# jabberjabberjabber/video-3d-pipeline

Hardware: AMD Instinct MI355X
Metric: 1080p_sbs_to_4k_depth_frames_per_s (higher is better)
Workload: dtype int16 (SGM) + f64 (guided filter sums; f32 depth in/out)

## Files before the change

### video-3d-pipeline_amd/csrc/v3d_common.h

```cpp
#pragma once
#include <hip/hip_runtime.h>
#include <stdint.h>
#include <stdio.h>
#include <stdarg.h>
#include "../../include/v3d_hip.h"

#define V3D_D 64
#define V3D_MAX_COST 32767
#define V3D_INVALID16 (-16)

void v3d_set_error(const char* fmt, ...);

struct v3d_lib_options {
    int gf_band1, gf_band2;
    int gf_tiled;
    int gf_fused;
    int gf_band;
    int gf_cols;
    int gf_int1;
    int corr_gather;
    int corr_fused;
};
extern v3d_lib_options g_v3d_opt;

#define V3D_HIP_CHECK(expr)                                                              \
    do {                                                                                 \
        hipError_t _e = (expr);                                                          \
        if (_e != hipSuccess) {                                                          \
            v3d_set_error("%s failed: %s (%s:%d)", #expr, hipGetErrorString(_e), __FILE__, __LINE__); \
            (void)hipGetLastError();    \
            return V3D_ERR_HIP;                                                          \
        }                                                                                \
    } while (0)

#define V3D_LAUNCH_CHECK()                                                               \
    do {                                                                                 \
        hipError_t _e = hipGetLastError();                                               \
        if (_e != hipSuccess) {                                                          \
            v3d_set_error("kernel launch failed: %s (%s:%d)", hipGetErrorString(_e), __FILE__, __LINE__); \
            return V3D_ERR_HIP;                                                          \
        }                                                                                \
    } while (0)

static inline int v3d_cdiv(int a, int b) { return (a + b - 1) / b; }

#ifdef __HIPCC__
typedef short v3d_s16x2 __attribute__((ext_vector_type(2)));
typedef unsigned short v3d_u16x2 __attribute__((ext_vector_type(2)));

__device__ __forceinline__ v3d_s16x2 as_s(uint32_t a) { return __builtin_bit_cast(v3d_s16x2, a); }
__device__ __forceinline__ v3d_u16x2 as_us(uint32_t a) { return __builtin_bit_cast(v3d_u16x2, a); }
__device__ __forceinline__ uint32_t as_u(v3d_s16x2 a) { return __builtin_bit_cast(uint32_t, a); }
__device__ __forceinline__ uint32_t as_u(v3d_u16x2 a) { return __builtin_bit_cast(uint32_t, a); }

__device__ __forceinline__ uint32_t pk_min(uint32_t a, uint32_t b) { return as_u(__builtin_elementwise_min(as_s(a), as_s(b))); }
__device__ __forceinline__ uint32_t pk_max(uint32_t a, uint32_t b) { return as_u(__builtin_elementwise_max(as_s(a), as_s(b))); }
__device__ __forceinline__ uint32_t pk_add(uint32_t a, uint32_t b) { return as_u((v3d_s16x2)(as_s(a) + as_s(b))); }
__device__ __forceinline__ uint32_t pk_sub(uint32_t a, uint32_t b) { return as_u((v3d_s16x2)(as_s(a) - as_s(b))); }
__device__ __forceinline__ uint32_t pk_add_sat(uint32_t a, uint32_t b) { return as_u(__builtin_elementwise_add_sat(as_s(a), as_s(b))); }
__device__ __forceinline__ uint32_t pk_subu_sat(uint32_t a, uint32_t b) { return as_u(__builtin_elementwise_sub_sat(as_us(a), as_us(b))); }
__device__ __forceinline__ uint32_t pk_minu(uint32_t a, uint32_t b) { return as_u(__builtin_elementwise_min(as_us(a), as_us(b))); }
__device__ __forceinline__ uint32_t pk_shr_u(uint32_t a, int n) { return as_u((v3d_u16x2)(as_us(a) >> (unsigned short)n)); }
__device__ __forceinline__ uint32_t pk_bcast(int v) { return ((uint32_t)v & 0xFFFFu) * 0x00010001u; }

__device__ __forceinline__ uint32_t alignbit(uint32_t hi, uint32_t lo, uint32_t sh) { return __builtin_amdgcn_alignbit(hi, lo, sh); }

#define V3D_DPP_QUAD(a, b, c, d) ((a) | ((b) << 2) | ((c) << 4) | ((d) << 6))
#define V3D_DPP_ROW_SHL(n) (0x100 + (n))
#define V3D_DPP_ROW_SHR(n) (0x110 + (n))
#define V3D_DPP_ROW_MIRROR 0x140
#define V3D_DPP_ROW_HALF_MIRROR 0x141

template <int CTRL>
__device__ __forceinline__ uint32_t dpp_mov(uint32_t old, uint32_t src)
{
    return (uint32_t)__builtin_amdgcn_update_dpp((int)old, (int)src, CTRL, 0xF, 0xF, false);
}
template <int CTRL>
__device__ __forceinline__ uint32_t dpp_xchg(uint32_t src)
{
    return (uint32_t)__builtin_amdgcn_update_dpp(0, (int)src, CTRL, 0xF, 0xF, true);
}
#ifndef V3D_NT
#define V3D_NT 1
#endif
typedef uint32_t v3d_u32x4 __attribute__((ext_vector_type(4)));
typedef uint32_t v3d_u32x2 __attribute__((ext_vector_type(2)));
__device__ __forceinline__ uint4 ld_stream(const uint4* p)
{
#if V3D_NT
    const v3d_u32x4 v = __builtin_nontemporal_load(reinterpret_cast<const v3d_u32x4*>(p));
    return make_uint4(v.x, v.y, v.z, v.w);
#else
    return *p;
#endif
}
__device__ __forceinline__ uint2 ld_stream(const uint2* p)
{
#if V3D_NT
    const v3d_u32x2 v = __builtin_nontemporal_load(reinterpret_cast<const v3d_u32x2*>(p));
    return make_uint2(v.x, v.y);
#else
    return *p;
#endif
}
__device__ __forceinline__ void st_stream(uint4* p, uint4 v)
{
#if V3D_NT
    v3d_u32x4 t = { v.x, v.y, v.z, v.w };
    __builtin_nontemporal_store(t, reinterpret_cast<v3d_u32x4*>(p));
#else
// ... 44 lines not shown
```

### video-3d-pipeline_amd/csrc/v3d_sgbm.hip

```cpp
#include "v3d_common.h"
#include <vector>
#include <string.h>
#include <type_traits>

#ifndef V3D_CK_NT
#define V3D_CK_NT 1
#endif
#ifndef V3D_C12
#define V3D_C12 1
#endif
#ifndef V3D_X_SPLIT
#define V3D_X_SPLIT 0
#endif
#define VOL_PX V3D_D
__host__ __device__ static inline size_t vol_row(int y, int W1) { return (size_t)y * W1 * V3D_D; }
__host__ __device__ static inline size_t vol_frame(int H, int W1) { return (size_t)H * W1 * V3D_D; }
#define C_PXB (V3D_C12 ? 96 : 128)
__host__ __device__ static inline size_t c_row(int y, int W1) { return (size_t)y * W1 * C_PXB; }
__host__ __device__ static inline size_t c_frame(int H, int W1) { return (size_t)H * W1 * C_PXB; }

#ifndef PF_BAND
#define PF_BAND 64
#endif
__global__ __launch_bounds__(256) void k_prefilter(const uint8_t* __restrict__ img1, const uint8_t* __restrict__ img2,
// ... 220 lines not shown
#pragma unroll
                for (int j = 0; j < NP; j++) V[i][j] = pr[j];
            }
#pragma unroll
            for (int j = 0; j < NP; j++) {
                const uint32_t c = bt_pair(U[0], U[1], U[2], V[0][j], V[1][j], V[2][j]);
                pix[j] = pl == 0 ? c : pix[j] + pk_shr_u(c, 2);
            }
            if (pl == 0) { if (NP == 4) asm volatile("" : "+v"(pix[0]), "+v"(pix[1]), "+v"(pix[NP - 2]), "+v"(pix[NP - 1]) :: "memory");
                           else asm volatile("" : "+v"(pix[0]), "+v"(pix[NP - 1]) :: "memory"); }
        }
        sPix[buf][col][dq] = Packer<NP>::go(pix);

        if (k + 1 < nrows && ld_any) stage(buf ^ 1, nr[buf ^ 1]);
        nr[buf ^ 1] = fetch(k + 3);
        __syncthreads();

        {
            uint32_t h[NP], w[NP];
            vec_unpack<NP>(sPix[buf][hc - 2][dq], h);
#pragma unroll
            for (int t = -1; t <= 2; t++) {
                vec_unpack<NP>(sPix[buf][hc + t][dq], w);
#pragma unroll
                for (int j = 0; j < NP; j++) h[j] += w[j];
            }
#pragma unroll
            for (int j = 0; j < NP; j++) { vs[j] += h[j] - ring[slot][j]; ring[slot][j] = h[j]; }
            const uint32_t st_row = k >= 4 ? (uint32_t)c_row(ys + k - 4, W1) : V3D_BUF_OOB;
            const uint32_t st_off = __builtin_elementwise_add_sat(st_col, st_row);
#if V3D_C12
            {
                uint32_t t[NP];
#pragma unroll
                for (int j = 0; j < NP; j++)
                    asm("v_bfi_b32 %0, %1, %2, %3" : "=v"(t[j]) : "s"(0xFFFu), "v"(vs[j]), "v"(vs[j] >> 4));
                const v3d_u32x3_a4 pk = { __builtin_amdgcn_perm(t[1], t[0], 0x04020100u), __builtin_amdgcn_perm(t[2], t[1], 0x05040201u),
                                          __builtin_amdgcn_perm(t[NP - 1], t[2], 0x06050402u) };
                __builtin_amdgcn_raw_buffer_store_b96(pk, rs_c, st_off, 0, V3D_NT ? 2 : 0);
            }
#else
            buf_store_stream(rs_c, st_off, Packer<NP>::go(vs));
#endif
        }
      }
    }
}

struct ChainArgs {
    const unsigned char* C; int16_t* S;
    int W1, H, W, nframes;
    int P1, P2;
    int uniq;
    uint32_t* wta;
    int xcd;
    int persist;
    int* ticket;
};

template <int LPP>
__device__ __forceinline__ uint32_t pk_hmin_lanes(uint32_t mn)
{
    uint32_t m1;
    asm("v_pk_min_u16 %0, %1, %1 op_sel:[0,1] op_sel_hi:[1,0]" : "=v"(m1) : "v"(mn));
    m1 = min(m1, dpp_xchg<V3D_DPP_QUAD(1, 0, 3, 2)>(m1));
    m1 = min(m1, dpp_xchg<V3D_DPP_QUAD(2, 3, 0, 1)>(m1));
    if (LPP >= 8) m1 = min(m1, dpp_xchg<V3D_DPP_ROW_HALF_MIRROR>(m1));
    if (LPP >= 16) m1 = min(m1, dpp_xchg<V3D_DPP_ROW_MIRROR>(m1));
    return m1;
}

template <int NP, int LPP>
__device__ __forceinline__ uint32_t chain_step(const uint32_t (&p)[NP], uint32_t delta, const uint32_t (&c)[NP],
                                               uint32_t (&L)[NP], uint32_t P1pk, uint32_t P2pk, bool first_lane, bool last_lane)
{
    const uint32_t MAXPK = 0x7FFF7FFFu;
    const uint32_t fill_prev = first_lane ? MAXPK : 0u, fill_next = last_lane ? MAXPK : 0u;
    const uint32_t prev = dpp_xchg<V3D_DPP_ROW_SHR(1)>(p[NP - 1]) | fill_prev;
    const uint32_t next = dpp_xchg<V3D_DPP_ROW_SHL(1)>(p[0]) | fill_next;
    uint32_t m[NP + 1];
    m[0] = alignbit(p[0], prev, 16);
#pragma unroll
    for (int i = 1; i < NP; i++) m[i] = alignbit(p[i], p[i - 1], 16);
    m[NP] = alignbit(next, p[NP - 1], 16);
    uint32_t mn = MAXPK;
#pragma unroll
    for (int i = 0; i < NP; i++) {
        uint32_t n = pk_add(pk_min(m[i], m[i + 1]), P1pk);
        L[i] = pk_sub(c[i], pk_subu_sat(delta, pk_min(p[i], n)));
        mn = pk_min(mn, L[i]);
    }
    return pk_add(pk_hmin_lanes<LPP>(mn), P2pk);
}

template <int NP, int LPP>
__device__ __forceinline__ uint32_t chain_delta(const uint32_t (&p)[NP], uint32_t P2pk)
{
    uint32_t mn = p[0];
#pragma unroll
    for (int i = 1; i < NP; i++) mn = pk_min(mn, p[i]);
    return pk_add(pk_hmin_lanes<LPP>(mn), P2pk);
}

#define WTA_ROWB 144

__device__ __forceinline__ uint32_t wta_word(int minS, int d16, int best) { return ((uint32_t)minS << 17) | ((uint32_t)(d16 + 16) << 6) | (uint32_t)best; }
__device__ __forceinline__ int wta_d16(uint32_t w) { return (int)((w >> 6) & 0x7FFu) - 16; }

__device__ __forceinline__ void wta_pixel(const unsigned char* srow, bool valid, int x, int y, int frame,
                                          const ChainArgs& a)
{
    uint32_t v[32];
#pragma unroll
    for (int q = 0; q < 8; q++) {
        const uint4 t = *reinterpret_cast<const uint4*>(srow + q * 16);
        v[4 * q] = t.x; v[4 * q + 1] = t.y; v[4 * q + 2] = t.z; v[4 * q + 3] = t.w;
    }
    uint32_t mpk = v[0];
#pragma unroll
    for (int i = 1; i < 32; i++) mpk = pk_minu(mpk, v[i]);
    const int minS = (int)min(mpk & 0xFFFFu, mpk >> 16);
    const uint32_t minpk = pk_bcast(minS), k64 = 0x00400040u;
    uint32_t kacc = 0xFFFFFFFFu;
#pragma unroll
    for (int i = 0; i < 32; i++) {
        uint32_t key;
        const uint32_t t = pk_subu_sat(v[i], minpk), dc = (uint32_t)(2 * i) | ((uint32_t)(2 * i + 1) << 16);
        asm("v_pk_mad_u16 %0, %1, %2, %3 clamp" : "=v"(key) : "v"(t), "v"(k64), "s"(dc));
        kacc = pk_minu(kacc, key);
    }
    const int best = (int)(min(kacc & 0xFFFFu, kacc >> 16) & 63u);
    const int uq = 100 - a.uniq, thr = minS * 100;
    int T1 = uq > 0 ? (thr + uq - 1) / uq : (thr > 0 ? 32768 : 0);
    T1 = min(T1, 32768);
    const uint32_t T1pk = pk_bcast(T1), one = 0x00010001u;
    uint32_t cntpk = 0;
#pragma unroll
    for (int i = 0; i < 32; i++) cntpk += pk_minu(pk_subu_sat(T1pk, v[i]), one);
    const int cnt = (int)(cntpk & 0xFFFFu) + (int)(cntpk >> 16);
    const unsigned short* s16 = reinterpret_cast<const unsigned short*>(srow);
    const int sm = best > 0 ? (int)s16[best - 1] : 0, sp = best < V3D_D - 1 ? (int)s16[best + 1] : 0;
    int cw = (minS < T1) ? 1 : 0;
    if (best > 0 && sm < T1) cw++;
    if (best < V3D_D - 1 && sp < T1) cw++;
    const bool ok = valid && (minS < V3D_MAX_COST) && (cnt <= cw);
    if (!valid) return;
    uint32_t word = 0u;
    if (ok) {
        int d16 = best * 16;
        if (best > 0 && best < V3D_D - 1) {
            const int den = max(sm + sp - 2 * minS, 1);
            d16 += ((sm - sp) * 16 + den) / (den * 2);
        }
        word = wta_word(minS, d16, best);
    }
    a.wta[((size_t)frame * a.H + y) * a.W + x + V3D_D] = word;
}

template <bool HORIZ, int XS, bool YREV, int MODE, int DPL>
__global__ __launch_bounds__(256) void k_chain(ChainArgs a)
{
    constexpr int NP = DPL / 2, LPP = 64 / DPL, PPW = DPL;
    constexpr int PF = 4;
    constexpr int BS = 64 / PPW;
    typedef typename VecT<DPL>::type Vec;
    static_assert(MODE != 2 || HORIZ, "the WTA tail rides on a horizontal direction");

    __shared__ __attribute__((aligned(16))) unsigned char sS[MODE == 2 ? 4 * 64 * WTA_ROWB : 16];

    const int lane = threadIdx.x & 63, wib = threadIdx.x >> 6;
    const int W1 = a.W1, H = a.H;
    const int NC = HORIZ ? H : (XS == 0 ? W1 : W1 + H - 1);
    const int groups = (NC + PPW - 1) / PPW;
    const int gw = blockIdx.x * 4 + wib;
    const int frame = gw / groups, grp = gw - frame * groups;
    if (frame >= a.nframes) return;

    const int sub = lane / LPP, dl = lane % LPP;
    const int c0 = grp * PPW, c1 = min(c0 + PPW, NC) - 1;
    const int c = c0 + sub;
    const bool cvalid = c <= c1;
    const int cc = min(c, c1);

    int tlo = 0, thi;
    if (HORIZ) thi = W1;
    else if (XS == 0) thi = H;
    else if (XS > 0) { tlo = max(0, H - 1 - c1); thi = min(H, W1 + H - 1 - c0); }
    else { tlo = max(0, c0 - (W1 - 1)); thi = min(H, c1 + 1); }

    const unsigned char* Cf = a.C + (size_t)frame * c_frame(H, W1) + c_lane_off<DPL>(dl);
    int16_t* Sf = a.S + (size_t)frame * vol_frame(H, W1) + dl * DPL;
    const int x0 = HORIZ ? 0 : (XS == 0 ? cc : (XS > 0 ? cc - (H - 1) : cc));

    auto pos = [&](int t, int& x, int& y) {
        if (HORIZ) { x = XS > 0 ? t : W1 - 1 - t; y = cc; }
        else { y = YREV ? H - 1 - t : t; x = x0 + XS * t; }
    };
    auto pix_off = [&](int t) -> int {
        int x, y; pos(t, x, y);
        x = min(max(x, 0), W1 - 1);
        return y * W1 + x;
    };

    const uint32_t P1pk = pk_bcast(a.P1), P2pk = pk_bcast(a.P2);
    const bool first_lane = dl == 0, last_lane = dl == LPP - 1;

    uint32_t p[NP];
#pragma unroll
    for (int i = 0; i < NP; i++) p[i] = 0;
// ... 28 lines not shown
                bool active = cvalid;
                if (!HORIZ && XS != 0) {
                    int x, y; pos(t, x, y);
                    active = cvalid && ((unsigned)x < (unsigned)W1);
#pragma unroll
                    for (int i = 0; i < NP; i++) L[i] = active ? L[i] : 0u;
                    nd = active ? nd : P2pk;
                }
#pragma unroll
                for (int i = 0; i < NP; i++) p[i] = L[i];
                delta = nd;
                if (MODE == 0) {
                    if (active) *reinterpret_cast<Vec*>(Sf + o) = Packer<NP>::go(L);
                } else {
#pragma unroll
                    for (int i = 0; i < NP; i++) sv[i] = pk_add_sat(sv[i], L[i]);
                    if (MODE == 1) {
                        if (active) *reinterpret_cast<Vec*>(Sf + o) = Packer<NP>::go(sv);
                    } else {
                        *reinterpret_cast<Vec*>(myS + (sub * BS + jj) * WTA_ROWB + dl * DPL * 2) = Packer<NP>::go(sv);
                    }
                }
            }
        }
        if (MODE == 2) {
            const int wsub = lane / BS, wj = lane % BS;
            const int t = tb + wj;
            const int y = c0 + wsub;
            const int x = XS > 0 ? t : W1 - 1 - t;
            const bool valid = (y <= c1) && (t < thi);
            wta_pixel(myS + lane * WTA_ROWB, valid, x, y, frame, a);
        }
    }
}

template <int DPL> struct HfC {
    typedef typename CRaw<DPL>::type Raw;
    static __device__ __forceinline__ const unsigned char* base(const unsigned char* C, int frame, int H, int W1, int row, int dl)
    {
        return C + (size_t)frame * c_frame(H, W1) + c_row(row, W1) + c_lane_off<DPL>(dl);
    }
    static __device__ __forceinline__ Raw load(const unsigned char* b, int x) { return c_load<DPL, !V3D_C12>(b + (size_t)x * C_PXB); }
};

template <int DPL>
__device__ __forceinline__ void hf_phase1(const unsigned char* Crow, uint32_t* ck, int nblk, int dl, uint32_t P1pk, uint32_t P2pk)
{
    constexpr int NP = DPL / 2, LPP = 64 / DPL, K = 64 / DPL;
    const bool first_lane = dl == 0, last_lane = dl == LPP - 1;
    uint32_t p[NP];
#pragma unroll
    for (int i = 0; i < NP; i++) p[i] = 0;
    uint32_t delta = P2pk;
    const int xend = (nblk - 1) * K;
    for (int xb = 0; xb < xend; xb += K) {
        typename HfC<DPL>::Raw cb[K];
#pragma unroll
        for (int jj = 0; jj < K; jj++) cb[jj] = HfC<DPL>::load(Crow, xb + jj);
#pragma unroll
        for (int jj = 0; jj < K; jj++) {
            uint32_t cv[NP], L[NP];
            vec_unpack<NP>(c_unpack(cb[jj], dl, P2pk), cv);
            delta = chain_step<NP, LPP>(p, delta, cv, L, P1pk, P2pk, first_lane, last_lane);
#pragma unroll
            for (int i = 0; i < NP; i++) p[i] = L[i];
        }
        uint32_t* c = ck + (size_t)(xb / K + 1) * NP * 64;
#pragma unroll
        for (int i = 0; i < NP; i++) { if (V3D_CK_NT) __builtin_nontemporal_store(p[i], c + i * 64); else c[i * 64] = p[i]; }
    }
}

template <int DPL, int PH>
__global__ __launch_bounds__(256, 4) void k_hfused(ChainArgs a, uint32_t* __restrict__ ckpt)
{
    constexpr int NP = DPL / 2, LPP = 64 / DPL, PPW = DPL, K = 64 / PPW;
    typedef typename VecT<DPL>::type Vec;
    __shared__ __attribute__((aligned(16))) unsigned char sS[4 * 64 * WTA_ROWB];

    const int lane = threadIdx.x & 63, wib = threadIdx.x >> 6;
    const int W1 = a.W1, H = a.H;
    const int groups = (H + PPW - 1) / PPW, total = groups * a.nframes;
    const int sub = lane / LPP, dl = lane % LPP;
    const int nblk = (W1 + K - 1) / K;
    const uint32_t P1pk = pk_bcast(a.P1), P2pk = pk_bcast(a.P2);
    const bool first_lane = dl == 0, last_lane = dl == LPP - 1;
    unsigned char* myS = sS + wib * 64 * WTA_ROWB;
    auto draw = [&]() -> int {
        int g = 0;
        if (lane == 0) g = atomicAdd(a.ticket, 1);
        return __builtin_amdgcn_readfirstlane(g);
    };
    int work = a.persist ? draw() : (a.xcd ? (int)xcd_linear(blockIdx.x, gridDim.x) : (int)blockIdx.x) * 4 + wib;
    for (;;) {
    if (work >= total) break;
    {
    const int frame = work / groups, grp = work - frame * groups;
    const int c0 = grp * PPW, c1 = min(c0 + PPW, H) - 1;
    const int cc = min(c0 + sub, c1);
    const unsigned char* Crow = HfC<DPL>::base(a.C, frame, H, W1, cc, dl);
    const int16_t* Srow = a.S + (size_t)frame * vol_frame(H, W1) + vol_row(cc, W1) + dl * DPL;
    uint32_t* ck = ckpt + ((size_t)frame * groups + grp) * nblk * NP * 64 + lane;
    if (PH & 1) hf_phase1<DPL>(Crow, ck, nblk, dl, P1pk, P2pk);

    uint32_t q[NP];
#pragma unroll
    for (int i = 0; i < NP; i++) q[i] = 0;
    uint32_t qdelta = P2pk;
    for (int blk = nblk - 1; blk >= 0; blk--) {
        const int x0 = blk * K;
        typename HfC<DPL>::Raw craw[K]; Vec cvv[K], svv[K];
#pragma unroll
        for (int j = 0; j < K; j++) {
            const int xj = min(x0 + j, W1 - 1);
            craw[j] = HfC<DPL>::load(Crow, xj);
            svv[j] = ld_stream(reinterpret_cast<const Vec*>(Srow + (size_t)xj * VOL_PX));
        }
        uint32_t p[NP], delta = P2pk;
#pragma unroll
        for (int i = 0; i < NP; i++) p[i] = 0;
        if (blk > 0) {
            const uint32_t* c = ck + (size_t)blk * NP * 64;
#pragma unroll
            for (int i = 0; i < NP; i++) p[i] = V3D_CK_NT ? __builtin_nontemporal_load(c + i * 64) : c[i * 64];
            delta = chain_delta<NP, LPP>(p, P2pk);
        }
        uint32_t L0[K][NP];
#pragma unroll
        for (int j = 0; j < K; j++) {
            uint32_t cv[NP];
            cvv[j] = c_unpack(craw[j], dl, P2pk);
            vec_unpack<NP>(cvv[j], cv);
            delta = chain_step<NP, LPP>(p, delta, cv, L0[j], P1pk, P2pk, first_lane, last_lane);
#pragma unroll
            for (int i = 0; i < NP; i++) p[i] = L0[j][i];
        }
#pragma unroll
        for (int jj = 0; jj < K; jj++) {
            const int j = K - 1 - jj;
            if (x0 + j < W1) {
                uint32_t cv[NP], sv[NP], L[NP];
                vec_unpack<NP>(cvv[j], cv);
                vec_unpack<NP>(svv[j], sv);
                qdelta = chain_step<NP, LPP>(q, qdelta, cv, L, P1pk, P2pk, first_lane, last_lane);
#pragma unroll
                for (int i = 0; i < NP; i++) { q[i] = L[i]; sv[i] = pk_add_sat(pk_add_sat(sv[i], L0[j][i]), L[i]); }
                *reinterpret_cast<Vec*>(myS + (sub * K + jj) * WTA_ROWB + dl * DPL * 2) = Packer<NP>::go(sv);
            }
        }
        {
            const int wsub = lane / K, wj = lane % K;
            const int x = x0 + K - 1 - wj, y = c0 + wsub;
            wta_pixel(myS + lane * WTA_ROWB, (y <= c1) && (x < W1), x, y, frame, a);
        }
    }
    }
    if (!a.persist) break;
    work = draw();
    }
}

template <int DPL>
__global__ __launch_bounds__(256, 8) void k_hscan(ChainArgs a, uint32_t* __restrict__ ckpt)
{
    constexpr int NP = DPL / 2, LPP = 64 / DPL, PPW = DPL, K = 64 / PPW;
    const int lane = threadIdx.x & 63, wib = threadIdx.x >> 6;
    const int W1 = a.W1, H = a.H;
    const int groups = (H + PPW - 1) / PPW;
    const int gw = (int)blockIdx.x * 4 + wib;
    const int frame = gw / groups, grp = gw - frame * groups;
    if (frame >= a.nframes) return;
    const int sub = lane / LPP, dl = lane % LPP;
    const int c0 = grp * PPW, c1 = min(c0 + PPW, H) - 1;
    const int cc = min(c0 + sub, c1);
    const int nblk = (W1 + K - 1) / K;
    uint32_t* ck = ckpt + ((size_t)frame * groups + grp) * nblk * NP * 64 + lane;
    hf_phase1<DPL>(HfC<DPL>::base(a.C, frame, H, W1, cc, dl), ck, nblk, dl, pk_bcast(a.P1), pk_bcast(a.P2));
}

#define VDD_RING 4
#define VDD_GRAN 34
#define VDD_SPIN_PER_ROW 64
#define VDD_SPIN_SLACK 4096

struct VddArgs {
    const unsigned char* C; int16_t* S;
    int W1, H, nframes, nstrips;
    int P1, P2;
    uint32_t seq;
    int spin_limit;
    unsigned long long* gran;
    int* err;
    int xcd;
};

template <int N>
__device__ __forceinline__ bool vdd_poll_n(const unsigned long long* g, const unsigned long long* gd, bool want_d,
                                           uint32_t tag, uint32_t (&v)[N], uint32_t& vd, int& budget)
{
    for (;;) {
        unsigned long long x[N], xd = (unsigned long long)tag << 32;
#pragma unroll
        for (int i = 0; i < N; i++) x[i] = __hip_atomic_load(g + i, __ATOMIC_RELAXED, __HIP_MEMORY_SCOPE_AGENT);
        if (want_d) xd = __hip_atomic_load(gd, __ATOMIC_RELAXED, __HIP_MEMORY_SCOPE_AGENT);
        bool ok = (uint32_t)(xd >> 32) == tag;
#pragma unroll
        for (int i = 0; i < N; i++) ok = ok && ((uint32_t)(x[i] >> 32) == tag);
        if (ok) {
// ... 533 lines not shown
}

__global__ __launch_bounds__(256) void k_ccl_apply(int16_t* __restrict__ img, int W, int H, int newVal, int maxSize,
                                                   const int* __restrict__ lab, const int* __restrict__ runs, const int* __restrict__ csz)
{
    const int y = blockIdx.x * 4 + (threadIdx.x >> 6), lane = threadIdx.x & 63;
    if (y >= H) return;
    const size_t fo = (size_t)blockIdx.z * W * H;
    const int* L = lab + fo;
    const int* rl = runs + fo + (size_t)y * W;
    const int row_end = (y + 1) * W;
    for (int k0 = 0; k0 < W; k0 += 64) {
        const int k = k0 + lane;
        const int s = k < W ? rl[k] : -1;
        const unsigned long long endm = __builtin_amdgcn_ballot_w64(s < 0);
        const int first_end = endm ? __builtin_ctzll(endm) : 64;
        if (lane < first_end) {
            const int r = ccl_find(L, s);
            if (csz[fo + r] <= maxSize) {
                img[fo + s] = (int16_t)newVal;
                for (int i = s + 1; i < row_end && L[i] == s; i++) img[fo + i] = (int16_t)newVal;
            }
        }
        if (first_end < 64) break;
    }
}

static int launch_speckles(int16_t* img, int W, int H, int frames, int newVal, int maxSize, int maxDiff, int32_t* ws, hipStream_t st)
{
    const int px = W * H;
    int* lab = ws; int* runs = ws + (size_t)px * frames; int* csz = ws + (size_t)px * frames * 2;
    hipLaunchKernelGGL(k_ccl_runs, dim3(v3d_cdiv(H, 4), 1, frames), dim3(256), 0, st, img, W, H, newVal, maxDiff, lab, runs, csz);
    hipLaunchKernelGGL(k_ccl_vmerge<0>, dim3(v3d_cdiv(W, 512), H - H / VM_BAND, frames), dim3(64), 0, st, img, W, H, newVal, maxDiff, lab);
    if (H / VM_BAND > 0) hipLaunchKernelGGL(k_ccl_vmerge<1>, dim3(v3d_cdiv(W, 512), H / VM_BAND, frames), dim3(64), 0, st, img, W, H, newVal, maxDiff, lab);
    hipLaunchKernelGGL(k_ccl_count, dim3(v3d_cdiv(H, 4), 1, frames), dim3(256), 0, st, W, H, maxSize, lab, runs, csz);
    hipLaunchKernelGGL(k_ccl_apply, dim3(v3d_cdiv(H, 4), 1, frames), dim3(256), 0, st, img, W, H, newVal, maxSize, lab, runs, csz);
    V3D_LAUNCH_CHECK();
    return V3D_OK;
}

__global__ __launch_bounds__(256) void k_c_export(const unsigned char* __restrict__ C, size_t npx, int P2, int16_t* __restrict__ out)
{
    const size_t i = (size_t)blockIdx.x * 256 + threadIdx.x, px = i >> 3;
    const int dl = (int)(i & 7);
    if (px >= npx) return;
    const uint4 v = c_unpack(*reinterpret_cast<const typename CRaw<8>::type*>(C + px * C_PXB + c_lane_off<8>(dl)), dl, pk_bcast(P2));
    *reinterpret_cast<uint4*>(out + px * V3D_D + 8 * dl) = v;
}

struct v3d_sgbm {
    v3d_sgbm_params prm;
    int device, maxW, maxH, maxB;
    int P1, P2, ftzero, uniq, d12;
    int dpl;
    uint4* rec;
    unsigned char* C;
    int16_t* S;
    uint32_t* wta;
    uint32_t* ckpt;
    unsigned long long* gran;
    size_t gran_bytes;
    int* vdd_err;
    uint32_t vdd_seq;
    int vdd_mode;
    int vdd_dpl;
    int cost_band;
    int vdd_xcd, cost_xcd, hf_xcd;
    int lrm_tiles;
    int hf_persist;
    int* hf_ticket;
    int vdd_mf4, vdd_mf8;
    int vdd_occ4, vdd_occ8, ncu;
    int reserve_cus;
    int vdd_launch_frames;
    int vdd_spin_limit;
    int* err_host;
    hipEvent_t vdd_done_ev;
    bool vdd_ev_recorded;
    bool hfused;
    int hsplit;
    int32_t* labels;
    size_t bytes;
    bool prof_on;
    int prof_calls;
    std::vector<hipEvent_t> prof_ev;
};

enum { ST_PREFILTER = 0, ST_COST, ST_V2, ST_D1, ST_D3, ST_H0, ST_V2R, ST_D1R, ST_D3R, ST_H4_WTA, ST_LRCHECK, ST_MEDIAN, ST_SPECKLE, V3D_NSTAGE };
static const char* const g_stage_names[V3D_NSTAGE] = { "prefilter", "cost", "chain_v2", "chain_d1", "chain_d3", "chain_h0",
    "chain_v2r", "chain_d1r", "chain_d3r", "chain_h4_wta", "lrcheck", "median", "speckles" };
#define V3D_PROF_MAX_CALLS 512

static inline void prof_mark(v3d_sgbm* h, int slot, hipStream_t stm)
{
    if (!h->prof_on || h->prof_calls >= V3D_PROF_MAX_CALLS) return;
    (void)hipEventRecord(h->prof_ev[(size_t)h->prof_calls * (V3D_NSTAGE + 1) + slot], stm);
}

extern "C" void v3d_sgbm_default_params(v3d_sgbm_params* p)
{
    p->minDisparity = 0; p->numDisparities = 64; p->blockSize = 5; p->P1 = 8 * 3 * 25; p->P2 = 32 * 3 * 25;
    p->disp12MaxDiff = 1; p->preFilterCap = 0; p->uniquenessRatio = 10; p->speckleWindowSize = 100;
    p->speckleRange = 32; p->mode = V3D_MODE_SGBM;
}

template <typename T> static int ws_alloc(T** p, size_t n, size_t* total)
// ... 31 lines not shown
    else if (is("vdd_xcd")) { if (value != 0 && value != 1) return bad(); h->vdd_xcd = value; }
    else if (is("hf_xcd")) { if (value != 0 && value != 1) return bad(); h->hf_xcd = value; }
    else if (is("hf_persist")) { if (value != 0 && value != 1) return bad(); h->hf_persist = value; }
    else if (is("lrm_tiles")) { if (value != 0 && value != 1) return bad(); h->lrm_tiles = value; }
    else if (is("reserve_cus")) { if (value < 0 || value > h->ncu) return bad(); h->reserve_cus = value; vdd_size_launches(h); }
    else if (is("vdd_spin_limit")) { if (value < -1) return bad(); h->vdd_spin_limit = value; }
    else if (is("vdd_launch_frames")) { if (value < 0) return bad(); h->vdd_launch_frames = value; }
    else { v3d_set_error("unknown option %s", key); return V3D_ERR_ARG; }
    return V3D_OK;
}
extern "C" int v3d_sgbm_get_option(const v3d_sgbm* h, const char* key, int* value)
{
    if (!h || !key || !value) { v3d_set_error("null argument"); return V3D_ERR_ARG; }
    auto is = [&](const char* k) { return strcmp(key, k) == 0; };
    if (is("lockstep")) *value = vdd_usable(h) ? 1 : 0;
    else if (is("hfused")) *value = h->hfused ? 1 : 0;
    else if (is("chain_dpl")) *value = h->dpl;
    else if (is("hsplit")) *value = h->hsplit;
    else if (is("vdd_dpl")) *value = h->vdd_dpl;
    else if (is("cost_band")) *value = h->cost_band;
    else if (is("cost_xcd")) *value = h->cost_xcd;
    else if (is("vdd_xcd")) *value = h->vdd_xcd;
    else if (is("hf_xcd")) *value = h->hf_xcd;
    else if (is("hf_persist")) *value = h->hf_persist;
    else if (is("lrm_tiles")) *value = h->lrm_tiles;
    else if (is("reserve_cus")) *value = h->reserve_cus;
    else if (is("vdd_spin_limit")) *value = h->vdd_spin_limit;
    else if (is("vdd_launch_frames")) *value = h->vdd_launch_frames;
    else if (is("vdd_frames_per_launch_dpl4")) *value = h->vdd_mf4;
    else if (is("vdd_frames_per_launch_dpl8")) *value = h->vdd_mf8;
    else { v3d_set_error("unknown option %s", key); return V3D_ERR_ARG; }
    return V3D_OK;
}

extern "C" int v3d_sgbm_create(const v3d_sgbm_params* prm, int device, int maxW, int maxH, int maxB, v3d_sgbm** out)
{
    if (!prm || !out) { v3d_set_error("null argument"); return V3D_ERR_ARG; }
    if (prm->minDisparity != 0 || prm->numDisparities != V3D_D || prm->blockSize != 5) {
        v3d_set_error("this build supports minDisparity=0, numDisparities=64, blockSize=5 (got %d, %d, %d)",
                      prm->minDisparity, prm->numDisparities, prm->blockSize);
        return V3D_ERR_UNSUPPORTED;
    }
    if (prm->mode != V3D_MODE_SGBM && prm->mode != V3D_MODE_HH) { v3d_set_error("unsupported mode %d", prm->mode); return V3D_ERR_UNSUPPORTED; }
    if (maxW <= V3D_D + 4 || maxH < 1 || maxB < 1) { v3d_set_error("bad geometry %dx%d batch %d", maxW, maxH, maxB); return V3D_ERR_ARG; }
    if ((size_t)maxW * maxH * V3D_D >= ((size_t)1 << 30)) { v3d_set_error("frame too large for 31-bit volume byte offsets"); return V3D_ERR_UNSUPPORTED; }
    V3D_HIP_CHECK(hipSetDevice(device));
    v3d_sgbm* h = new v3d_sgbm();
    h->prof_on = false; h->prof_calls = 0;
    h->prm = *prm; h->device = device; h->maxW = maxW; h->maxH = maxH; h->maxB = maxB;
    h->P1 = prm->P1 > 0 ? prm->P1 : 2;
    h->P2 = prm->P2 > 0 ? prm->P2 : 5; if (h->P2 < h->P1 + 1) h->P2 = h->P1 + 1;
    h->ftzero = (prm->preFilterCap > 15 ? prm->preFilterCap : 15) | 1;
    h->uniq = prm->uniquenessRatio >= 0 ? prm->uniquenessRatio : 10;
    h->d12 = prm->disp12MaxDiff > 0 ? prm->disp12MaxDiff : 1;
    if (2 * h->P2 + 25 * (2 * h->ftzero + 63) >= 32767 || h->ftzero > 31) {
        const int p2 = h->P2; delete h;
        v3d_set_error("P2=%d / preFilterCap exceed the int16 range of the packed SGM recurrence (need 2*P2 + 25*(2*ftzero+63) < 32767)", p2);
        return V3D_ERR_UNSUPPORTED;
    }
    h->dpl = 4;
    const size_t px = (size_t)maxW * maxH * maxB, vol = vol_frame(maxH, maxW - V3D_D) * maxB;
    h->bytes = 0;
    int rc = 0;
    rc |= ws_alloc(&h->rec, px, &h->bytes);
    rc |= ws_alloc(&h->C, c_frame(maxH, maxW - V3D_D) * maxB, &h->bytes);   rc |= ws_alloc(&h->S, vol, &h->bytes);
    rc |= ws_alloc(&h->wta, px, &h->bytes); rc |= ws_alloc(&h->labels, px * 3, &h->bytes);
    {
        const int W1m = maxW - V3D_D;
        const size_t c4 = (size_t)v3d_cdiv(maxH, 4) * v3d_cdiv(W1m, 16) * 64 * 3, c8 = (size_t)v3d_cdiv(maxH, 8) * v3d_cdiv(W1m, 8) * 64 * 5;
        rc |= ws_alloc(&h->ckpt, (c4 > c8 ? c4 : c8) * maxB, &h->bytes);
    }
    h->hfused = true; h->hsplit = V3D_X_SPLIT;
    {
        h->vdd_dpl = 0;
        const int nstrips_max = v3d_cdiv(maxW - V3D_D, 64);
        const size_t ng = (size_t)maxB * nstrips_max * 2 * VDD_RING * VDD_GRAN;
        rc |= ws_alloc(&h->gran, ng, &h->bytes); h->gran_bytes = ng * sizeof(unsigned long long);
        rc |= ws_alloc(&h->vdd_err, 64, &h->bytes);
        h->hf_ticket = h->vdd_err ? h->vdd_err + 32 : nullptr;
        if (!rc) { (void)hipMemset(h->gran, 0, ng * sizeof(unsigned long long)); (void)hipMemset(h->vdd_err, 0, 64 * sizeof(int)); }
        h->err_host = nullptr;
        if (!rc && hipHostMalloc((void**)&h->err_host, 64, hipHostMallocDefault) != hipSuccess) { h->err_host = nullptr; rc = 1; }
        if (h->err_host) *h->err_host = 0;
        h->vdd_done_ev = nullptr; h->vdd_ev_recorded = false;
        if (!rc && hipEventCreateWithFlags(&h->vdd_done_ev, hipEventDisableTiming) != hipSuccess) { h->vdd_done_ev = nullptr; rc = 1; }
        h->vdd_seq = 1;
        h->vdd_mode = 1;
        h->reserve_cus = 0; h->vdd_spin_limit = 0; h->vdd_launch_frames = 0;
        int b4 = 0, b8 = 0, ncu = 0;
        (void)hipOccupancyMaxActiveBlocksPerMultiprocessor(&b4, k_vdd<4, true>, 1024, 0);
        (void)hipOccupancyMaxActiveBlocksPerMultiprocessor(&b8, k_vdd<8, true>, 1024, 0);
        (void)hipDeviceGetAttribute(&ncu, hipDeviceAttributeMultiprocessorCount, device);
        h->vdd_occ4 = b4 > 2 ? 2 : b4; h->vdd_occ8 = b8 > 2 ? 2 : b8; h->ncu = ncu;
        vdd_size_launches(h);
    }
    h->lrm_tiles = 0;
    h->hf_persist = 1;
    h->vdd_xcd = 0; h->hf_xcd = 0; h->cost_xcd = 1;
    h->cost_band = 90;
    if (rc) { v3d_sgbm_destroy(h); return V3D_ERR_HIP; }
    *out = h;
    return V3D_OK;
}

extern "C" void v3d_sgbm_destroy(v3d_sgbm* h)
{
// ... 38 lines not shown
    const int mf4 = vdd_frames_per_launch(h, 4, W1), mf8 = vdd_frames_per_launch(h, 8, W1);
    const int dpl = h->vdd_dpl ? h->vdd_dpl : (n <= mf4 ? 4 : 8);
    const int mf = h->vdd_launch_frames > 0 ? h->vdd_launch_frames : dpl == 8 ? (mf8 > 0 ? mf8 : 1) : (mf4 > 0 ? mf4 : 1);
    const int nl = v3d_cdiv(n, mf), per = v3d_cdiv(n, nl);
    for (int f0 = 0; f0 < n; f0 += per) {
        VddArgs v;
        const int nf = n - f0 < per ? n - f0 : per;
        v.C = h->C + (size_t)f0 * c_frame(H, W1); v.S = h->S + (size_t)f0 * vol_frame(H, W1);
        v.W1 = W1; v.H = H; v.nframes = nf; v.nstrips = v3d_cdiv(W1, 16 * dpl); v.P1 = h->P1; v.P2 = h->P2;
        v.seq = (h->vdd_seq++) & 0xFFFFFu;
        if (v.seq == 0) {
            (void)hipMemsetAsync(h->gran, 0, h->gran_bytes, st);
            v.seq = (h->vdd_seq++) & 0xFFFFFu;
        }
        v.gran = h->gran; v.err = h->vdd_err; v.xcd = h->vdd_xcd;
        v.spin_limit = h->vdd_spin_limit != 0 ? h->vdd_spin_limit : VDD_SPIN_PER_ROW * H + VDD_SPIN_SLACK;
        const dim3 grid(v.nstrips * nf), block(1024);
        if (dpl == 8) { if (rev) hipLaunchKernelGGL((k_vdd<8, true>), grid, block, 0, st, v); else hipLaunchKernelGGL((k_vdd<8, false>), grid, block, 0, st, v); }
        else { if (rev) hipLaunchKernelGGL((k_vdd<4, true>), grid, block, 0, st, v); else hipLaunchKernelGGL((k_vdd<4, false>), grid, block, 0, st, v); }
    }
}

static int lockstep_state(const v3d_sgbm* h)
{
    if (h->err_host && *(volatile int*)h->err_host != 0) {
        v3d_set_error("a lock-step SGM pass of an earlier call timed out (%d workgroups): its output was set to INVALID; "
                      "call v3d_sgbm_set_lockstep(h, 0) and recompute", *(volatile int*)h->err_host);
        return V3D_ERR_LOCKSTEP;
    }
    return V3D_OK;
}

static int run_sgbm(v3d_sgbm* h, const uint8_t* left, const uint8_t* right, int n, int W, int H, int pitch,
                    size_t frame_stride, int16_t* out, int last_stage, hipStream_t st)
{
    int rc = check_geometry(h, n, W, H, pitch);
    if (rc) return rc;
    if (!left || !right || !out) { v3d_set_error("null image pointer"); return V3D_ERR_ARG; }
    if ((rc = lockstep_state(h)) != V3D_OK) return rc;
    const int W1 = W - V3D_D;
    const int px = W * H;

    prof_mark(h, ST_PREFILTER, st);
    hipLaunchKernelGGL(k_prefilter, dim3(v3d_cdiv(W, 252), v3d_cdiv(H, PF_BAND), n), dim3(256), 0, st, left, right, W, H, pitch, frame_stride, h->ftzero, h->rec);
    prof_mark(h, ST_COST, st);
    constexpr int COST_OUT = CostGeo<V3D_COST_LPC>::OUT;
    hipLaunchKernelGGL((k_cost<V3D_COST_LPC>), dim3(v3d_cdiv(W1, COST_OUT), v3d_cdiv(H, h->cost_band), n), dim3(512), 0, st, h->rec, W, H, W1, h->cost_band, h->P2, h->C, h->cost_xcd);
    V3D_LAUNCH_CHECK();
    prof_mark(h, ST_V2, st);
    if (last_stage == 1) return V3D_OK;

    ChainArgs a;
    a.C = h->C; a.S = h->S; a.W1 = W1; a.H = H; a.W = W; a.nframes = n; a.P1 = h->P1; a.P2 = h->P2; a.uniq = h->uniq;
    a.wta = h->wta; a.xcd = h->hf_xcd; a.persist = 0; a.ticket = h->hf_ticket;
    const bool use_vdd = vdd_usable(h) && H < 4095;
    if (use_vdd) {
        launch_vdd(h, n, W1, H, false, st);
        prof_mark(h, ST_D1, st);
        prof_mark(h, ST_D3, st);
        V3D_HIP_CHECK(hipEventRecord(h->vdd_done_ev, st));
        h->vdd_ev_recorded = true;
    } else {
    launch_chain<false, 0, false, 0>(h, a, st);
    prof_mark(h, ST_D1, st);
    launch_chain<false, 1, false, 1>(h, a, st);
    prof_mark(h, ST_D3, st);
    launch_chain<false, -1, false, 1>(h, a, st);
    }
    prof_mark(h, ST_H0, st);
    if (!h->hfused) launch_chain<true, 1, false, 1>(h, a, st);
    prof_mark(h, ST_V2R, st);
    if (h->prm.mode == V3D_MODE_HH) {
        if (use_vdd) {
            launch_vdd(h, n, W1, H, true, st);
            prof_mark(h, ST_D1R, st); prof_mark(h, ST_D3R, st);
            V3D_HIP_CHECK(hipEventRecord(h->vdd_done_ev, st));
        } else {
            launch_chain<false, 0, true, 1>(h, a, st);
            prof_mark(h, ST_D1R, st);
            launch_chain<false, -1, true, 1>(h, a, st);
            prof_mark(h, ST_D3R, st);
            launch_chain<false, 1, true, 1>(h, a, st);
        }
    } else { prof_mark(h, ST_D1R, st); prof_mark(h, ST_D3R, st); }
    prof_mark(h, ST_H4_WTA, st);
    if (h->hfused) {
        const dim3 g4(v3d_cdiv(v3d_cdiv(H, 4) * n, 4)), g8(v3d_cdiv(v3d_cdiv(H, 8) * n, 4));
        if (h->hsplit) {
            if (h->dpl == 4) { hipLaunchKernelGGL(k_hscan<4>, g4, dim3(256), 0, st, a, h->ckpt); hipLaunchKernelGGL((k_hfused<4, 2>), g4, dim3(256), 0, st, a, h->ckpt); }
            else { hipLaunchKernelGGL(k_hscan<8>, g8, dim3(256), 0, st, a, h->ckpt); hipLaunchKernelGGL((k_hfused<8, 2>), g8, dim3(256), 0, st, a, h->ckpt); }
        } else {
            dim3 l4 = g4, l8 = g8;
            if (h->hf_persist) {
                a.persist = h->hf_persist;
                V3D_HIP_CHECK(hipMemsetAsync(h->hf_ticket, 0, sizeof(int), st));
                const unsigned res = (unsigned)h->ncu * 4u;
                if (l4.x > res) l4.x = res;
                if (l8.x > res) l8.x = res;
            }
            if (h->dpl == 4) hipLaunchKernelGGL((k_hfused<4, 3>), l4, dim3(256), 0, st, a, h->ckpt);
            else hipLaunchKernelGGL((k_hfused<8, 3>), l8, dim3(256), 0, st, a, h->ckpt);
            a.persist = 0;
        }
    } else
        launch_chain<true, -1, false, 2>(h, a, st);
    V3D_LAUNCH_CHECK();
// ... 130 lines not shown
```

Baseline: 2513.

## Streamline WTA pixel arithmetic and restructure fused horizontal SGM block loop

Replaces the per-pixel integer division for the uniqueness threshold with a host-precomputed magic multiply, and the subpixel division with a short restoring-division sequence. It also computes the uniqueness count with shift-based packed ops and makes the stores branchless. The fused horizontal chain now runs a peeled partial-width block followed by full blocks with no clamping, walking the row with pointers. The checkpoint for block 0 is written as zeros so that every block loads its checkpoint without a branch. These changes aim to cut ALU and divergence cost in the hot WTA path, at the risk of small numerical differences if the magic constants are wrong for some uniqueness values.

Result: faster. 2546, median of 6 (+1.3%).

```diff
diff --git a/video-3d-pipeline_amd/csrc/v3d_common.h b/video-3d-pipeline_amd/csrc/v3d_common.h
--- a/video-3d-pipeline_amd/csrc/v3d_common.h
+++ b/video-3d-pipeline_amd/csrc/v3d_common.h
@@ -45,6 +45,36 @@
 static inline int v3d_cdiv(int a, int b) { return (a + b - 1) / b; }
 
 #ifdef __HIPCC__
+#define V3D_HD __host__ __device__
+#else
+#define V3D_HD
+#endif
+V3D_HD static inline void v3d_t1_magic(int uq, uint32_t* mul, int* shift)
+{
+    int c = 0;
+    while ((1 << c) < uq) c++;
+    *shift = 23 + c;
+    *mul = (uint32_t)((((uint64_t)1 << *shift) + (uint64_t)uq - 1) / (uint64_t)uq);
+}
+V3D_HD static inline int v3d_t1_ceil(int minS, int uq, uint32_t mul, int shift)
+{
+    const uint32_t n = ((uint32_t)minS * 100u + (uint32_t)(uq - 1)) & 0xFFFFFFu;
+    return (int)(((uint64_t)n * (mul & 0xFFFFFFu)) >> shift);
+}
+V3D_HD static inline int v3d_subpix_q(int a, int b)
+{
+    const int den = a + b > 1 ? a + b : 1, num = (a - b) * 16 + den;
+    const uint32_t step = (uint32_t)(1 - 32 * den);
+    uint32_t R = (uint32_t)(num < 0 ? -num : num) << 4, t;
+    t = R + (step << 3); R = t < R ? t : R;
+    t = R + (step << 2); R = t < R ? t : R;
+    t = R + (step << 1); R = t < R ? t : R;
+    t = R + step; R = t < R ? t : R;
+    const int qm = (int)(R & 15u);
+    return num < 0 ? -qm : qm;
+}
+
+#ifdef __HIPCC__
 typedef short v3d_s16x2 __attribute__((ext_vector_type(2)));
 typedef unsigned short v3d_u16x2 __attribute__((ext_vector_type(2)));
 
@@ -57,6 +87,7 @@
 __device__ __forceinline__ uint32_t pk_max(uint32_t a, uint32_t b) { return as_u(__builtin_elementwise_max(as_s(a), as_s(b))); }
 __device__ __forceinline__ uint32_t pk_add(uint32_t a, uint32_t b) { return as_u((v3d_s16x2)(as_s(a) + as_s(b))); }
 __device__ __forceinline__ uint32_t pk_sub(uint32_t a, uint32_t b) { return as_u((v3d_s16x2)(as_s(a) - as_s(b))); }
+__device__ __forceinline__ uint32_t pk_subu(uint32_t a, uint32_t b) { return as_u((v3d_u16x2)(as_us(a) - as_us(b))); }
 __device__ __forceinline__ uint32_t pk_add_sat(uint32_t a, uint32_t b) { return as_u(__builtin_elementwise_add_sat(as_s(a), as_s(b))); }
 __device__ __forceinline__ uint32_t pk_subu_sat(uint32_t a, uint32_t b) { return as_u(__builtin_elementwise_sub_sat(as_us(a), as_us(b))); }
 __device__ __forceinline__ uint32_t pk_minu(uint32_t a, uint32_t b) { return as_u(__builtin_elementwise_min(as_us(a), as_us(b))); }
diff --git a/video-3d-pipeline_amd/csrc/v3d_sgbm.hip b/video-3d-pipeline_amd/csrc/v3d_sgbm.hip
--- a/video-3d-pipeline_amd/csrc/v3d_sgbm.hip
+++ b/video-3d-pipeline_amd/csrc/v3d_sgbm.hip
@@ -296,6 +296,7 @@
     int W1, H, W, nframes;
     int P1, P2;
     int uniq;
+    uint32_t t1_mul; int t1_shift;
     uint32_t* wta;
     int xcd;
     int persist;
@@ -365,40 +366,39 @@
     for (int i = 1; i < 32; i++) mpk = pk_minu(mpk, v[i]);
     const int minS = (int)min(mpk & 0xFFFFu, mpk >> 16);
     const uint32_t minpk = pk_bcast(minS), k64 = 0x00400040u;
-    uint32_t kacc = 0xFFFFFFFFu;
+    uint32_t kacc = 0xFFFFFFFFu, key[32];
+#pragma unroll
+    for (int i = 0; i < 32; i++) key[i] = pk_subu_sat(v[i], minpk);
 #pragma unroll
     for (int i = 0; i < 32; i++) {
-        uint32_t key;
-        const uint32_t t = pk_subu_sat(v[i], minpk), dc = (uint32_t)(2 * i) | ((uint32_t)(2 * i + 1) << 16);
-        asm("v_pk_mad_u16 %0, %1, %2, %3 clamp" : "=v"(key) : "v"(t), "v"(k64), "s"(dc));
-        kacc = pk_minu(kacc, key);
-    }
+        const uint32_t dc = (uint32_t)(2 * i) | ((uint32_t)(2 * i + 1) << 16);
+        asm("v_pk_mad_u16 %0, %1, %2, %3 clamp" : "=v"(key[i]) : "v"(key[i]), "v"(k64), "s"(dc));
+    }
+#pragma unroll
+    for (int i = 0; i < 32; i++) kacc = pk_minu(kacc, key[i]);
     const int best = (int)(min(kacc & 0xFFFFu, kacc >> 16) & 63u);
-    const int uq = 100 - a.uniq, thr = minS * 100;
-    int T1 = uq > 0 ? (thr + uq - 1) / uq : (thr > 0 ? 32768 : 0);
-    T1 = min(T1, 32768);
-    const uint32_t T1pk = pk_bcast(T1), one = 0x00010001u;
+    const int uq = 100 - a.uniq;
+    int t1q = v3d_t1_ceil(minS, uq, a.t1_mul, a.t1_shift);
+    asm volatile("" : "+v"(t1q));
+    const int T1 = min(uq > 0 ? t1q : min(minS, 1) << 15, 32768);
+    const uint32_t T1pk = pk_bcast(T1);
     uint32_t cntpk = 0;
 #pragma unroll
-    for (int i = 0; i < 32; i++) cntpk += pk_minu(pk_subu_sat(T1pk, v[i]), one);
+    for (int i = 0; i < 32; i += 2) cntpk += pk_shr_u(pk_subu(v[i], T1pk), 15) + pk_shr_u(pk_subu(v[i + 1], T1pk), 15);
     const int cnt = (int)(cntpk & 0xFFFFu) + (int)(cntpk >> 16);
     const unsigned short* s16 = reinterpret_cast<const unsigned short*>(srow);
+    const bool inner = best > 0 && best < V3D_D - 1;
     const int sm = best > 0 ? (int)s16[best - 1] : 0, sp = best < V3D_D - 1 ? (int)s16[best + 1] : 0;
     int cw = (minS < T1) ? 1 : 0;
     if (best > 0 && sm < T1) cw++;
     if (best < V3D_D - 1 && sp < T1) cw++;
-    const bool ok = valid && (minS < V3D_MAX_COST) && (cnt <= cw);
-    if (!valid) return;
-    uint32_t word = 0u;
-    if (ok) {
-        int d16 = best * 16;
-        if (best > 0 && best < V3D_D - 1) {
-            const int den = max(sm + sp - 2 * minS, 1);
-            d16 += ((sm - sp) * 16 + den) / (den * 2);
-        }
-        word = wta_word(minS, d16, best);
-    }
-    a.wta[((size_t)frame * a.H + y) * a.W + x + V3D_D] = word;
+    const bool ok = (minS < V3D_MAX_COST) && (cnt <= cw);
+    int subpix = v3d_subpix_q(sm - minS, sp - minS);
+    asm volatile("" : "+v"(subpix));
+    uint32_t word = wta_word(minS, best * 16 + (inner ? subpix : 0), best);
+    asm volatile("" : "+v"(word));
+    word = ok ? word : 0u;
+    if (valid) a.wta[((size_t)frame * a.H + y) * a.W + x + V3D_D] = word;
 }
 
 template <bool HORIZ, int XS, bool YREV, int MODE, int DPL>
@@ -533,6 +533,8 @@
 #pragma unroll
     for (int i = 0; i < NP; i++) p[i] = 0;
     uint32_t delta = P2pk;
+#pragma unroll
+    for (int i = 0; i < NP; i++) { if (V3D_CK_NT) __builtin_nontemporal_store(p[i], ck + i * 64); else ck[i * 64] = p[i]; }
     const int xend = (nblk - 1) * K;
     for (int xb = 0; xb < xend; xb += K) {
         typename HfC<DPL>::Raw cb[K];
@@ -552,11 +554,49 @@
     }
 }
 
+template <int DPL, bool FULL>
+__device__ __forceinline__ void hf_block(const unsigned char* Cb, const int16_t* Sb, int nvalid, uint32_t (&p)[DPL / 2], uint32_t delta,
+                                         uint32_t (&q)[DPL / 2], uint32_t& qdelta, unsigned char* Sl, int dl, uint32_t P1pk, uint32_t P2pk)
+{
+    constexpr int NP = DPL / 2, LPP = 64 / DPL, K = 64 / DPL;
+    typedef typename VecT<DPL>::type Vec;
+    const bool first_lane = dl == 0, last_lane = dl == LPP - 1;
+    typename HfC<DPL>::Raw craw[K]; Vec cvv[K], svv[K];
+#pragma unroll
+    for (int j = 0; j < K; j++) {
+        const int xj = FULL ? j : min(j, nvalid - 1);
+        craw[j] = HfC<DPL>::load(Cb, xj);
+        svv[j] = ld_stream(reinterpret_cast<const Vec*>(Sb + (size_t)xj * VOL_PX));
+    }
+    uint32_t L0[K][NP];
+#pragma unroll
+    for (int j = 0; j < K; j++) {
+        uint32_t cv[NP];
+        cvv[j] = c_unpack(craw[j], dl, P2pk);
+        vec_unpack<NP>(cvv[j], cv);
+        delta = chain_step<NP, LPP>(p, delta, cv, L0[j], P1pk, P2pk, first_lane, last_lane);
+#pragma unroll
+        for (int i = 0; i < NP; i++) p[i] = L0[j][i];
+    }
+#pragma unroll
+    for (int jj = 0; jj < K; jj++) {
+        const int j = K - 1 - jj;
+        if (FULL || j < nvalid) {
+            uint32_t cv[NP], sv[NP], L[NP];
+            vec_unpack<NP>(cvv[j], cv);
+            vec_unpack<NP>(svv[j], sv);
+            qdelta = chain_step<NP, LPP>(q, qdelta, cv, L, P1pk, P2pk, first_lane, last_lane);
+#pragma unroll
+            for (int i = 0; i < NP; i++) { q[i] = L[i]; sv[i] = pk_add_sat(pk_add_sat(sv[i], L0[j][i]), L[i]); }
+            *reinterpret_cast<Vec*>(Sl + jj * WTA_ROWB) = Packer<NP>::go(sv);
+        }
+    }
+}
+
 template <int DPL, int PH>
 __global__ __launch_bounds__(256, 4) void k_hfused(ChainArgs a, uint32_t* __restrict__ ckpt)
 {
     constexpr int NP = DPL / 2, LPP = 64 / DPL, PPW = DPL, K = 64 / PPW;
-    typedef typename VecT<DPL>::type Vec;
     __shared__ __attribute__((aligned(16))) unsigned char sS[4 * 64 * WTA_ROWB];
 
     const int lane = threadIdx.x & 63, wib = threadIdx.x >> 6;
@@ -565,7 +605,6 @@
     const int sub = lane / LPP, dl = lane % LPP;
     const int nblk = (W1 + K - 1) / K;
     const uint32_t P1pk = pk_bcast(a.P1), P2pk = pk_bcast(a.P2);
-    const bool first_lane = dl == 0, last_lane = dl == LPP - 1;
     unsigned char* myS = sS + wib * 64 * WTA_ROWB;
     auto draw = [&]() -> int {
         int g = 0;
@@ -588,53 +627,27 @@
 #pragma unroll
     for (int i = 0; i < NP; i++) q[i] = 0;
     uint32_t qdelta = P2pk;
-    for (int blk = nblk - 1; blk >= 0; blk--) {
+    const unsigned char* Cb = Crow + (size_t)(nblk - 1) * K * C_PXB;
+    const int16_t* Sb = Srow + (size_t)(nblk - 1) * K * VOL_PX;
+    unsigned char* Sl = myS + sub * K * WTA_ROWB + dl * DPL * 2;
+    const int wsub = min(lane / K, c1 - c0), wj = lane % K, y = c0 + wsub;
+    const unsigned char* Wl = myS + (wsub * K + wj) * WTA_ROWB;
+    auto block = [&](int blk, auto full) {
+        constexpr bool FULL = decltype(full)::value;
         const int x0 = blk * K;
-        typename HfC<DPL>::Raw craw[K]; Vec cvv[K], svv[K];
-#pragma unroll
-        for (int j = 0; j < K; j++) {
-            const int xj = min(x0 + j, W1 - 1);
-            craw[j] = HfC<DPL>::load(Crow, xj);
-            svv[j] = ld_stream(reinterpret_cast<const Vec*>(Srow + (size_t)xj * VOL_PX));
-        }
-        uint32_t p[NP], delta = P2pk;
-#pragma unroll
-        for (int i = 0; i < NP; i++) p[i] = 0;
-        if (blk > 0) {
-            const uint32_t* c = ck + (size_t)blk * NP * 64;
-#pragma unroll
-            for (int i = 0; i < NP; i++) p[i] = V3D_CK_NT ? __builtin_nontemporal_load(c + i * 64) : c[i * 64];
-            delta = chain_delta<NP, LPP>(p, P2pk);
-        }
-        uint32_t L0[K][NP];
-#pragma unroll
-        for (int j = 0; j < K; j++) {
-            uint32_t cv[NP];
-            cvv[j] = c_unpack(craw[j], dl, P2pk);
-            vec_unpack<NP>(cvv[j], cv);
-            delta = chain_step<NP, LPP>(p, delta, cv, L0[j], P1pk, P2pk, first_lane, last_lane);
-#pragma unroll
-            for (int i = 0; i < NP; i++) p[i] = L0[j][i];
-        }
-#pragma unroll
-        for (int jj = 0; jj < K; jj++) {
-            const int j = K - 1 - jj;
-            if (x0 + j < W1) {
-                uint32_t cv[NP], sv[NP], L[NP];
-                vec_unpack<NP>(cvv[j], cv);
-                vec_unpack<NP>(svv[j], sv);
-                qdelta = chain_step<NP, LPP>(q, qdelta, cv, L, P1pk, P2pk, first_lane, last_lane);
-#pragma unroll
-                for (int i = 0; i < NP; i++) { q[i] = L[i]; sv[i] = pk_add_sat(pk_add_sat(sv[i], L0[j][i]), L[i]); }
-                *reinterpret_cast<Vec*>(myS + (sub * K + jj) * WTA_ROWB + dl * DPL * 2) = Packer<NP>::go(sv);
-            }
-        }
-        {
-            const int wsub = lane / K, wj = lane % K;
-            const int x = x0 + K - 1 - wj, y = c0 + wsub;
-            wta_pixel(myS + lane * WTA_ROWB, (y <= c1) && (x < W1), x, y, frame, a);
-        }
-    }
+        uint32_t p[NP];
+        const uint32_t* c = ck + (size_t)blk * NP * 64;
+#pragma unroll
+        for (int i = 0; i < NP; i++) p[i] = V3D_CK_NT ? __builtin_nontemporal_load(c + i * 64) : c[i * 64];
+        const uint32_t delta = chain_delta<NP, LPP>(p, P2pk);
+        hf_block<DPL, FULL>(Cb, Sb, FULL ? K : W1 - x0, p, delta, q, qdelta, Sl, dl, P1pk, P2pk);
+        const int x = x0 + K - 1 - wj;
+        wta_pixel(Wl, FULL || x < W1, x, y, frame, a);
+        Cb -= K * C_PXB; Sb -= K * VOL_PX;
+    };
+    int blk = nblk - 1;
+    if (W1 % K) block(blk--, std::false_type());
+    for (; blk >= 0; blk--) block(blk, std::true_type());
     }
     if (!a.persist) break;
     work = draw();
@@ -1274,6 +1287,7 @@
     v3d_sgbm_params prm;
     int device, maxW, maxH, maxB;
     int P1, P2, ftzero, uniq, d12;
+    uint32_t t1_mul; int t1_shift;
     int dpl;
     uint4* rec;
     unsigned char* C;
@@ -1411,6 +1425,8 @@
     h->P2 = prm->P2 > 0 ? prm->P2 : 5; if (h->P2 < h->P1 + 1) h->P2 = h->P1 + 1;
     h->ftzero = (prm->preFilterCap > 15 ? prm->preFilterCap : 15) | 1;
     h->uniq = prm->uniquenessRatio >= 0 ? prm->uniquenessRatio : 10;
+    h->t1_mul = 0; h->t1_shift = 0;
+    if (h->uniq < 100) v3d_t1_magic(100 - h->uniq, &h->t1_mul, &h->t1_shift);
     h->d12 = prm->disp12MaxDiff > 0 ? prm->disp12MaxDiff : 1;
     if (2 * h->P2 + 25 * (2 * h->ftzero + 63) >= 32767 || h->ftzero > 31) {
         const int p2 = h->P2; delete h;
@@ -1555,6 +1571,7 @@
 
     ChainArgs a;
     a.C = h->C; a.S = h->S; a.W1 = W1; a.H = H; a.W = W; a.nframes = n; a.P1 = h->P1; a.P2 = h->P2; a.uniq = h->uniq;
+    a.t1_mul = h->t1_mul; a.t1_shift = h->t1_shift;
     a.wta = h->wta; a.xcd = h->hf_xcd; a.persist = 0; a.ticket = h->hf_ticket;
     const bool use_vdd = vdd_usable(h) && H < 4095;
     if (use_vdd) {
```
